# Polochon-street/bliss-rs

Measured on AMD Instinct MI355X. Metric: songs/sec (3-min 22 050 Hz f32) at 1/2/4/8 GPU; HBM GB/s vs roofline, higher is better.
Workload: dtype f32; 1 GPU; configs[1]: batch of 1024 synthetic 3969000-sample (3-min) white-noise f32 PCM buffers per GPU, full 23-feature descriptor set (FeaturesVersion 2); songs_per_gpu=1024, songs_total=1024, features=23, parallelism=single GPU

## Files before the change

bliss-rs_amd/csrc/blissgpu.hip:

```cpp
#include <math.h>
#include <stdio.h>
#include <stdlib.h>
#include <string.h>

#include <algorithm>
#include <atomic>
#include <chrono>
#include <deque>
#include <mutex>
#include <string>
#include <vector>

#include "ctx.hpp"
#include "forest.hpp"

using namespace bg;

namespace {
thread_local std::string g_last_error;

const char* const kKernelNames[K_COUNT] = {
    "fft512_kernel",     "onset_kernel",      "beat_kernel",   "stft8192_kernel", "tune_select_kernel",
    "tune_pass2_kernel", "tune_final_kernel", "chroma_kernel",     "summary_kernel", "assemble_kernel", "pairwise_kernel", "set_distance_kernel", "song_to_song_kernel", "synth_kernel", "rolloff_fix_kernel",
    "dedup_next_kernel", "dedup_walk_kernel", "knn_scan_kernel", "knn_merge_kernel",
// ... 1368 lines not shown
    return BLISSGPU_OK;
}

int blissgpu_debug_fetch(blissgpu_ctx* c, int what, uint32_t song, void* dst, uint64_t max_elems, uint64_t* n_elems) {
    if (!c || !dst) return fail(BLISSGPU_ERR_INVALID, "blissgpu_debug_fetch", "NULL argument");
    CTX_ENTER(c, "blissgpu_debug_fetch");
    if (what == BLISSGPU_DEBUG_FILTER_BANK) {
        if (song > (uint32_t)N_TUNING) return fail(BLISSGPU_ERR_INVALID, "blissgpu_debug_fetch", "tuning slot must be 0..100");
        const uint64_t n = (uint64_t)BANK_ROWS * BANK_PITCH;
        if (n_elems) *n_elems = n;
        const uint64_t k = std::min(n, max_elems);
        HIP_TRY(hipStreamSynchronize(c->stream));
        if (k) HIP_TRY(hipMemcpy(dst, c->chroma_bank + (size_t)song * n, k * sizeof(double), hipMemcpyDeviceToHost));
        return BLISSGPU_OK;
    }
    size_t pos = c->last_songs.size();
    for (size_t i = 0; i < c->last_songs.size(); i++)
        if (c->last_songs[i].row == song) { pos = i; break; }
    if (pos == c->last_songs.size()) return fail(BLISSGPU_ERR_INVALID, "blissgpu_debug_fetch", "no such song in the last chunk");
    HIP_TRY(hipStreamSynchronize(c->stream));
    const SongDesc& d = c->last_songs[pos];
    const Workspace& w = c->last_ws;
    const void* src = nullptr;
    uint64_t n = 0, esz = 4;
    const uint64_t runs = d.ok ? (d.n_b >= (uint32_t)BT_STEP ? (d.n_b - BT_STEP) / BT_STEP + 1 : 0) : 0;
    switch (what) {
        case BLISSGPU_DEBUG_CENTROID: src = w.centroid + d.t_off; n = d.n_t; break;
        case BLISSGPU_DEBUG_ROLLOFF: src = w.rolloff + d.t_off; n = d.n_t; break;
        case BLISSGPU_DEBUG_FLATNESS: src = w.flatness + d.t_off; n = d.n_t; break;
        case BLISSGPU_DEBUG_FLUX: src = w.flux + d.b_off; n = d.n_b; break;
        case BLISSGPU_DEBUG_THRESHOLDED: src = w.thresholded + d.b_off; n = d.n_b; break;
        case BLISSGPU_DEBUG_RUN_BPM: src = w.run_bpm + pos * w.runs_pitch; n = runs; break;
        case BLISSGPU_DEBUG_RUN_COUNT: src = w.run_cnt + pos * w.runs_pitch; n = runs; break;
        case BLISSGPU_DEBUG_SPECTROGRAM: src = w.spec + d.c_off * (size_t)CBINS_PAD; n = (uint64_t)d.n_c * CBINS_PAD; break;
        case BLISSGPU_DEBUG_ENERGY256: src = w.e256 + d.e_off; n = d.n_e; break;
        case BLISSGPU_DEBUG_CROSSINGS256: src = w.zc256 + d.e_off; n = d.n_e; break;
        case BLISSGPU_DEBUG_PITCH_HIST: src = w.hist100 + pos * N_TUNING; n = N_TUNING; break;
        case BLISSGPU_DEBUG_CHROMA:
        case BLISSGPU_DEBUG_INTERVAL:
            if (!w.dbg_chroma || !w.dbg_interval)
                return fail(BLISSGPU_ERR_INVALID, "blissgpu_debug_fetch", "set BLISSGPU_OPT_DEBUG_CHROMA before the analysis");
            esz = 8;
            if (what == BLISSGPU_DEBUG_CHROMA) { src = w.dbg_chroma + d.c_off * 12; n = (uint64_t)d.n_c * 12; }
            else { src = w.dbg_interval + pos * 10; n = 10; }
            break;
        default: return fail(BLISSGPU_ERR_INVALID, "blissgpu_debug_fetch", "unknown tap");
    }
    if (!d.ok) n = 0;
    if (n_elems) *n_elems = n;
    const uint64_t k = std::min(n, max_elems);
    if (k) HIP_TRY(hipMemcpy(dst, src, k * esz, hipMemcpyDeviceToHost));
    return BLISSGPU_OK;
}

}
```

bliss-rs_amd/csrc/internal.hpp:

```cpp
#pragma once
#include <hip/hip_runtime.h>
#include <stdint.h>

#include <vector>

namespace bg {

constexpr uint32_t SAMPLE_RATE = 22050;
constexpr int W512 = 512;
constexpr int HOP_T = 128;
constexpr int HOP_B = 256;
constexpr int W8192 = 8192;
constexpr int HOP_C = 2205;
constexpr int CBINS = W8192 / 2 + 1;
constexpr int CBINS_PAD = 4128;
constexpr int BANK_PITCH = CBINS_PAD;
constexpr int BANK_ROWS = 12;
constexpr int LOUD_W = 1024;
constexpr int MIN_SAMPLES = 8192;
constexpr int N_TUNING = 100;
constexpr int PIP_LO = 57, PIP_HI = 1483;
constexpr int PIP_MAX_PER_FRAME = 714;
constexpr int CAND_BUDGET_PER_FRAME = 48;
#ifndef COARSE_SHIFT
#define COARSE_SHIFT 17
#endif
constexpr uint32_t COARSE_LOW_MASK = (1u << COARSE_SHIFT) - 1u;
constexpr int H1_BINS = 1 << (31 - COARSE_SHIFT);
constexpr int BT_WINLEN = 512, BT_STEP = 128, BT_LAGLEN = 128;
constexpr int BT_PRE_STRIDE = 264;
constexpr int F512_TILE = 512;
constexpr int CH_TILE = 64;
constexpr int STFT_TILE = 16;

struct SongDesc {
    uint64_t pcm_off;
    uint64_t n;
    uint64_t t_off;
    uint64_t b_off;
    uint64_t c_off;
    uint64_t e_off;
    uint32_t n_t;
    uint32_t n_b;
    uint32_t n_f;
    uint32_t n_c;
    uint32_t n_e;
    uint32_t n_l;
    uint32_t row;
    uint32_t ok;
};

struct RollFix {
    float* mags;
    uint32_t cap;
};
constexpr float ROLLOFF_UNPROVEN = -1.0f;

struct TuningState {
    uint32_t n_peaks;
    uint32_t b_lo, b_hi;
    uint32_t below;
    uint32_t n_cand;
    int32_t tuning_idx;
    uint32_t cand_off;
    uint32_t cand_cap;
};

struct TempoState {
    float tempo;
    uint32_t n_bpms;
};

struct DeviceTables {
    const float2* tw8192;
    const float2* tw512;
    const float* hann8192;
    const float* hannz512;
    const double* chroma_bank;
    const float* bt_rwv;
    const float* bt_dfwv;
};

// ... 57 lines not shown
    size_t roll_fix_bytes;
};

struct Batch {
    const float* pcm;
    const SongDesc* songs;
    uint32_t n_songs;
    const uint32_t* pfx_f;
    const uint32_t* pfx_c;
    const uint32_t* pfx_ct;
    const uint32_t* pfx_cw;
    uint32_t tiles_f, tiles_c, tiles_ct, tiles_cw;
    uint64_t total_b;
    uint32_t max_nb;
    uint32_t max_nt;
};

void launch_fft512(const Batch&, const Workspace&, const DeviceTables&, hipStream_t, bool rolloff_exact_all = false, bool seq_flux = false);
void launch_rolloff_fix(const Batch&, const Workspace&, uint64_t total_t, hipStream_t);
void launch_onset(const Batch&, const Workspace&, hipStream_t);
void launch_beat(const Batch&, const Workspace&, const DeviceTables&, hipStream_t);
void launch_beat_acf(const Batch&, const Workspace&, const DeviceTables&, hipStream_t);
void launch_beat_track(const Batch&, const Workspace&, const DeviceTables&, hipStream_t);
void launch_stft8192(const Batch&, const Workspace&, const DeviceTables&, hipStream_t, int shape = 0);
struct SongRange { uint32_t s0, s1, ct0, ct1, cw0, cw1; };
void launch_tune_select(const Batch&, const Workspace&, hipStream_t, const SongRange* r = nullptr);
void launch_tune_pass2(const Batch&, const Workspace&, hipStream_t, const SongRange* r = nullptr);
void launch_tune_final(const Batch&, const Workspace&, hipStream_t, const SongRange* r = nullptr);
void launch_chroma(const Batch&, const Workspace&, const DeviceTables&, hipStream_t, const SongRange* r = nullptr);
void launch_summary(const Batch&, const Workspace&, hipStream_t);
void launch_finalize(const Batch&, const Workspace&, uint32_t features_version, float* d_out, int32_t* d_status,
                     int32_t* dbg_tuning, uint32_t* dbg_nbpms, hipStream_t);
void launch_chroma_bank(double* bank, hipStream_t);
void launch_pcm_convert(const void* in, int sample_format, uint32_t channels, float* out, uint64_t frames, hipStream_t st);
struct SwrPlan;
hipError_t launch_resample(const void* in, int sample_format, uint32_t channels, uint64_t frames, const SwrPlan& plan,
                           const float* d_bank, float* out, uint64_t n_out, hipStream_t st);
void launch_pair_distance(const float* a, const float* b, uint32_t d, int metric, const float* d_M, float* out, hipStream_t st);
void launch_set_distance(const float* seeds, uint32_t n_seeds, const float* cand, uint64_t n, uint32_t d, int metric,
                         const float* M, float* dist, uint32_t* keys, uint32_t* idx, uint32_t* nan_flag, hipStream_t st);
hipError_t sort_pairs_u32(void* tmp, size_t* tmp_bytes, uint32_t* keys_in, uint32_t* keys_out, uint32_t* vals_in,
                          uint32_t* vals_out, uint32_t n, hipStream_t st, uint32_t* sync = nullptr, uint32_t max_coresident = 0);
void launch_song_to_song(const float* seeds, uint32_t n_seeds, const float* cand, uint32_t n, uint32_t d, int metric,
                         const float* M, uint32_t* order, unsigned long long* slots, uint32_t* sync, uint32_t grid,
                         hipStream_t st);
void launch_dedup_next(const float* x, uint64_t n, uint32_t d, const uint32_t* seq, uint32_t len, const uint32_t* meta,
                       int metric, const float* M, float thr, uint32_t* next, uint32_t* bad, hipStream_t st);
void launch_dedup_walk(const float* x, uint64_t n, uint32_t d, const uint32_t* seq, uint32_t len, const uint32_t* meta,
                       int metric, const float* M, float thr, const uint32_t* next, uint32_t* kept, uint64_t* n_kept,
                       uint32_t* nan_flag, uint32_t* bad, hipStream_t st);
struct KnnPlan {
    uint32_t cap;
    uint32_t qb;
    uint32_t n_split;
    uint32_t blocks_per_split;
    uint32_t grid_qb;
    uint64_t part_keys;
};
KnnPlan knn_plan(uint64_t q, uint64_t n, uint32_t k, int n_cus);
void launch_knn_scan(const float* Q, uint64_t q, const float* X, uint32_t n, uint32_t d, int metric, const float* M,
                     int m_is_diag, const uint32_t* skip, uint32_t k, const KnnPlan& p, unsigned long long* part,
                     uint32_t* nan_flag, uint32_t* bad_flag, hipStream_t st);
void launch_knn_merge(const unsigned long long* part, uint64_t q, uint32_t k, const KnnPlan& p, uint32_t* idx, float* dist,
                      hipStream_t st);
constexpr int GROUP_KNN_SEED_TILE = 32;
struct GroupKnnItem {
// ... 37 lines not shown
```

bliss-rs_amd/csrc/kernels_chroma.hip:

```cpp
#include <float.h>
#include <stdlib.h>

#include <type_traits>

#include "device_utils.hpp"
#include "fft_r16.hpp"
#include "internal.hpp"

namespace bg {

typedef double double4_t __attribute__((ext_vector_type(4)));

__device__ __forceinline__ double tuning_of_slot(int slot) {
    return slot >= N_TUNING ? 0.0 : (-50.0 + (100.0 * 0.01 * (double)slot)) / 100.0;
}

__global__ __launch_bounds__(256) void chroma_bank_kernel(double* __restrict__ bank) {
#pragma clang fp contract(off)
    const int slot = blockIdx.y;
    const int k = blockIdx.x * 256 + threadIdx.x;
    if (k >= BANK_PITCH) return;
    double* out = bank + (size_t)slot * BANK_ROWS * BANK_PITCH;
    if (k >= CBINS) {
        for (int r = 0; r < BANK_ROWS; r++) out[(size_t)r * BANK_PITCH + k] = 0.0;
// ... 381 lines not shown
            split_pair_sq(v[R16(j)], (j == 0 && t == 0) ? v[R16(0)] : zm, w, sq_k, sq_m);
            m_lo[j] = mag_from_sq(sq_k);
            m_hi[j] = mag_from_sq(sq_m);
            mx = fmaxf(mx, fmaxf(m_lo[j], m_hi[j]));
        }
        if (t == 0) {
            m_mid = mag_from_sq(split_one_sq(v[R16(8)], v[R16(8)], mk(0.0f, -1.0f)));
            mx = fmaxf(mx, m_mid);
        }
        const bool has_next = fi + 1 < STFT_FRAMES_PER_WG && f + STFT_GROUP < sd.n_c;
        if (has_next) load_frame(f + STFT_GROUP, v);
        mx = wave_max_dpp(mx);
        if constexpr (NARROW) __syncthreads();
        float* mags = reinterpret_cast<float*>(lds);
        float* mags_top = mags + MAGS_TOP_W - 4096;
#pragma unroll
        for (int j = 0; j < 8; j++) {
            mags[t + 256 * j] = m_lo[j];
            if (j == 0 && t == 0) mags_top[4096] = m_hi[0];
            else mags[4096 - (t + 256 * j)] = m_hi[j];
        }
        if (t == 0) mags[2048] = m_mid;
        if (t >= 1 && t < CBINS_PAD - 4096) mags_top[4096 + t] = 0.0f;
        {
            int slot = t >> 6;
            asm volatile("" : "+v"(slot));
            if (lane_id() == 0) red[slot] = mx;
        }
        if (t == 0) peak_count = 0;
        TRACE(10);
        __syncthreads();
        TRACE(11);
        auto store_row = [&]() {
            const __amdgpu_buffer_rsrc_t r_row = __builtin_amdgcn_make_buffer_rsrc(
                (void*)(spec + (sd.c_off + f) * (size_t)CBINS_PAD), 0, CBINS_PAD * 4, 0x00020000);
            const u32x4_t* mags4 = reinterpret_cast<const u32x4_t*>(lds);
#pragma unroll
            for (int i = 0; i < 5; i++) {
                const int q = t + 256 * i;
                if (i < 4 || q < CBINS_PAD / 4) {
                    const u32x4_t val = i < 4 ? mags4[q] : mags4[q - 1024 + MAGS_TOP_W / 4];
                    __builtin_amdgcn_raw_buffer_store_b128(val, r_row, 16u * (uint32_t)q, 0, 2);
                }
            }
        };
        store_row();
        mx = fmaxf(fmaxf(red[0], red[1]), fmaxf(red[2], red[3]));
        if (t == 0) frame_max[sd.c_off + f] = mx;
        if (!have_base) {
            if (t == 0) {
                const uint32_t top = coarse_bin((double)mx);
                lhist_base = top > (uint32_t)(LHIST_BINS * 3 / 4) ? top - (uint32_t)(LHIST_BINS * 3 / 4) : 0u;
            }
            have_base = true;
            __syncthreads();
        }
        TRACE(12);
        const uint32_t lbase = lhist_base;
        __builtin_amdgcn_s_setprio(2);
        const double ref = 0.1 * (double)mx;
        const float thr = ref_floor_f32(ref);
        {
            uint32_t hits = 0;
#pragma unroll
            for (int h = 0; h < 2; h++) {
                float sb3[3], se3[3], sa3[3];
#pragma unroll
                for (int q = 0; q < 3; q++) {
                    const int c = t + 256 * (3 * h + q);
                    sb3[q] = mags[c > 0 ? c - 1 : 0];
                    se3[q] = mags[c];
                    sa3[q] = mags[c + 1];
                }
#pragma unroll
                for (int q = 0; q < 3; q++) {
                    const int j = 3 * h + q, c = t + 256 * j;
                    const uint32_t in_range = (256 * j >= PIP_LO && 256 * j + 255 <= PIP_HI) ? 1u : (uint32_t)(c >= PIP_LO) & (uint32_t)(c <= PIP_HI);
                    const uint32_t pk = in_range & (uint32_t)(sa3[q] <= se3[q]) & (uint32_t)(sb3[q] < se3[q]) & (uint32_t)(se3[q] > thr);
                    hits |= pk << j;
                }
            }
            const uint32_t mine = (uint32_t)__popc(hits);
            const uint32_t incl = wave_scan_incl_u32_dpp(mine);
            uint32_t wbase = 0;
            if (lane_id() == 63) wbase = atomicAdd(&peak_count, incl);
            uint32_t pos = (uint32_t)__builtin_amdgcn_readlane((int)wbase, 63) + incl - mine;
#pragma unroll
            for (int j = 0; j < 6; j++)
                if ((hits >> j) & 1u) peak_list[pos++] = (uint16_t)(t + 256 * j);
            TRACE(13);
            __syncthreads();
            TRACE(14);
            const uint32_t n_peaks = peak_count;
            uint32_t* __restrict__ recs = peak_rec + (sd.c_off + f) * (size_t)PIP_MAX_PER_FRAME;
            if (t == 0) peak_cnt[sd.c_off + f] = n_peaks;
            int c_next = t < n_peaks ? (int)peak_list[t] : PIP_LO;
            for (uint32_t i = t; i < n_peaks; i += 256) {
                const int c = c_next;
                const float sb = mags[c - 1], se = mags[c], sa = mags[c + 1];
                c_next = i + 256 < n_peaks ? (int)peak_list[i + 256] : PIP_LO;
                int pb;
                const uint32_t b = peak_classify(sb, se, sa, ref, c, &pb), rel = b - lbase;
                recs[i] = peak_record(b, pb, c);
                if (rel < (uint32_t)LHIST_BINS) atomicAdd(&lhist[rel], 1u);
                else atomicAdd(&hist[b], 1u);
            }
        }
        __builtin_amdgcn_s_setprio(0);
        if (has_next) {
            load_window();
#pragma unroll
            for (int n1 = 0; n1 < 16; n1++) v[n1] = v[n1] * win[n1];
        }
        TRACE(15);
        __syncthreads();
        TRACE(16);
    }
    TRACE_FLUSH();
    if (have_base) {
        const uint32_t lbase = lhist_base;
        for (int i = t; i < LHIST_BINS; i += 256) {
            const uint32_t c = lhist[i];
            if (c) atomicAdd(&hist[lbase + i], c);
        }
    }
}

// ... 88 lines not shown

__global__ __launch_bounds__(256) void tune_pass2_kernel(const SongDesc* __restrict__ songs, uint32_t n_songs,
                                                         const uint32_t* __restrict__ pfx_ct,
                                                         const float* __restrict__ spec,
                                                         const float* __restrict__ frame_max,
                                                         const uint32_t* __restrict__ peak_rec,
                                                         const uint32_t* __restrict__ peak_cnt,
                                                         TuningState* __restrict__ tuning,
                                                         uint32_t* __restrict__ hist100,
                                                         double* __restrict__ cand_mag,
                                                         uint8_t* __restrict__ cand_pb, uint32_t first_tile) {
    __shared__ uint32_t hist[N_TUNING];
    __shared__ uint32_t slow_list[4][P2_SLOW_CAP];
    const uint32_t bx = blockIdx.x + first_tile;
    const uint32_t s = find_segment(pfx_ct, n_songs, bx);
    const SongDesc sd = songs[s];
    const uint32_t tile = bx - pfx_ct[s];
    const int tid = threadIdx.x, lane = lane_id(), wave = wave_id();
    TuningState* ts = tuning + s;
    const uint32_t b_lo = ts->b_lo, b_hi = ts->b_hi;
    if (ts->n_peaks == 0) return;
    const uint32_t cand_off = ts->cand_off;
    const uint32_t cand_cap = ts->cand_cap;
    const bool pooled = cand_cap != 0;
    if (tid < N_TUNING) hist[tid] = 0;
    __syncthreads();
    uint32_t n_slow = 0;

    auto flush = [&]() {
        for (uint32_t i = lane; i < n_slow; i += WAVE) {
            const uint32_t e = slow_list[wave][i];
            const int c = (int)(e & 0xFFFFu);
            const uint32_t f = tile * CH_TILE + wave + 4 * (e >> 16);
            const float* row = spec + (sd.c_off + f) * (size_t)CBINS_PAD;
            const double ref = 0.1 * (double)frame_max[sd.c_off + f];
            double mag, pitch;
            if (pip_peak_core(row[c - 1], row[c], row[c + 1], ref, c, &mag, &pitch)) {
                const uint32_t b = coarse_bin(mag);
                if (b > b_hi) {
                    atomicAdd(&hist[pitch_bin(pitch)], 1u);
                } else if (b >= b_lo) {
                    const uint32_t slot = atomicAdd(&ts->n_cand, 1u);
                    if (pooled && slot < cand_cap) {
                        cand_mag[cand_off + slot] = mag;
                        cand_pb[cand_off + slot] = (uint8_t)pitch_bin(pitch);
                    }
                }
            }
        }
        __builtin_amdgcn_wave_barrier();
        n_slow = 0;
    };
    uint32_t n_rec_next = 0;
    {
        const uint32_t f0 = tile * CH_TILE + wave;
        if (f0 < sd.n_c) n_rec_next = peak_cnt[sd.c_off + f0];
    }
    for (int i = 0; i < P2_FRAMES_PER_WAVE; i++) {
        const uint32_t f = tile * CH_TILE + wave + 4 * i;
        if (f >= sd.n_c) break;
        const uint32_t n_rec = n_rec_next < (uint32_t)PIP_MAX_PER_FRAME ? n_rec_next : (uint32_t)PIP_MAX_PER_FRAME;
        if (i + 1 < P2_FRAMES_PER_WAVE && f + 4 < sd.n_c) n_rec_next = peak_cnt[sd.c_off + f + 4];
        const uint32_t* __restrict__ recs = peak_rec + (sd.c_off + f) * (size_t)PIP_MAX_PER_FRAME;
        if (n_slow + PIP_MAX_PER_FRAME > P2_SLOW_CAP) flush();
        for (uint32_t j0 = 0; j0 < n_rec; j0 += 4 * WAVE) {
            uint32_t r4[4];
#pragma unroll
            for (int u = 0; u < 4; u++) {
                const uint32_t j = j0 + WAVE * u + lane;
                r4[u] = j < n_rec ? recs[j] : 0xFFFFFFFFu;
            }
#pragma unroll
            for (int u = 0; u < 4; u++) {
                if (j0 + WAVE * u >= n_rec) break;
                const uint32_t j = j0 + WAVE * u + lane;
                bool slow = false;
                uint32_t c = 0;
                if (j < n_rec) {
                    const uint32_t r = r4[u];
                    const uint32_t b = r >> 18, pbf = (r >> 11) & 0x7Fu;
                    c = r & 0x7FFu;
                    if (b > b_hi) {
                        if (pbf) atomicAdd(&hist[pbf - 1], 1u);
                        else slow = true;
                    } else if (b >= b_lo) {
                        slow = true;
                    }
                }
                const uint64_t mask = __ballot(slow);
                if (mask) {
                    if (slow) slow_list[wave][n_slow + (uint32_t)__popcll(mask & ((1ull << lane) - 1ull))] = ((uint32_t)i << 16) | c;
                    n_slow += (uint32_t)__popcll(mask);
                }
            }
        }
    }
// ... 69 lines not shown
    __shared__ unsigned long long s_min_gt;
    const uint32_t s = blockIdx.x + first_song;
    const int tid = threadIdx.x;
    TuningState* ts = tuning + s;
    const SongDesc sd = songs[s];
    if (!sd.ok || ts->n_peaks == 0) return;
    const uint32_t total = ts->n_peaks, nc = ts->n_cand;
    const uint32_t r_lo = (total - 1) / 2, r_hi = total - 1 - r_lo;
    const uint32_t k_lo = r_lo - ts->below, k_hi = r_hi - ts->below;
    const uint32_t b_lo = ts->b_lo, b_hi = ts->b_hi;
    const bool pooled = ts->cand_cap != 0 && nc == ts->cand_cap;
    const double* v = cand_mag + ts->cand_off;
    const uint8_t* pb = cand_pb + ts->cand_off;

    auto for_each = [&](auto&& fn) {
        if (pooled) {
            for (uint32_t i0 = tid; i0 < nc; i0 += 8 * 256) {
                double m8[8];
                int b8[8];
#pragma unroll
                for (int u = 0; u < 8; u++) {
                    const uint32_t i = i0 + 256u * u;
                    m8[u] = i < nc ? v[i] : 0.0;
                    b8[u] = i < nc ? (int)pb[i] : 0;
                }
#pragma unroll
                for (int u = 0; u < 8; u++)
                    if (i0 + 256u * u < nc) fn(m8[u], b8[u]);
            }
        } else {
            for (uint32_t f = 0; f < sd.n_c; f++) {
                const uint32_t n_rec_raw = peak_cnt[sd.c_off + f];
                const uint32_t n_rec = n_rec_raw < (uint32_t)PIP_MAX_PER_FRAME ? n_rec_raw : (uint32_t)PIP_MAX_PER_FRAME;
                const uint32_t* __restrict__ recs = peak_rec + (sd.c_off + f) * (size_t)PIP_MAX_PER_FRAME;
                const float* __restrict__ row = spec + (sd.c_off + f) * (size_t)CBINS_PAD;
                const double ref = 0.1 * (double)frame_max[sd.c_off + f];
                for (uint32_t j = tid; j < n_rec; j += 256) {
                    const uint32_t r = recs[j], b = r >> 18;
                    if (b < b_lo || b > b_hi) continue;
                    const int c = (int)(r & 0x7FFu);
                    double mag, pitch;
                    if (pip_peak_core(row[c - 1], row[c], row[c + 1], ref, c, &mag, &pitch)) fn(mag, pitch_bin(pitch));
                }
            }
        }
    };

    const uint64_t key_lo = block_radix_select(for_each, k_lo, hist, &s_digit, &s_rank, s_wave);
    uint64_t key_hi = key_lo;
    if (k_hi != k_lo) {
        if (tid == 0) { s_cnt_le = 0; s_min_gt = ~0ull; }
        __syncthreads();
        uint32_t cnt = 0;
        unsigned long long mn = ~0ull;
        for_each([&](double mag, int) {
            const uint64_t k = f64_key(mag);
            if (k <= key_lo) cnt++;
            else if (k < mn) mn = k;
        });
        atomicAdd(&s_cnt_le, cnt);
        atomicMin(&s_min_gt, mn);
        __syncthreads();
        if (s_cnt_le <= k_hi) key_hi = s_min_gt;
    }
    double thr;
    {
#pragma clang fp contract(off)
        const double lo = key_f64(key_lo), hi = key_f64(key_hi);
        thr = lo + (hi - lo) / 2.0;
    }
    __syncthreads();
    if (tid < N_TUNING) hist[tid] = hist100[(size_t)s * N_TUNING + tid];
    __syncthreads();
    for_each([&](double mag, int bin) {
        if (mag >= thr) atomicAdd(&hist[bin], 1u);
// ... 11 lines not shown
    const uint32_t s0 = r ? r->s0 : 0, s1 = r ? r->s1 : b.n_songs;
    if (s1 <= s0) return;
    hipLaunchKernelGGL(tune_final_kernel, dim3(s1 - s0), dim3(256), 0, st, b.songs, w.tuning, w.hist100,
                       w.cand_mag, w.cand_pb, w.spec, w.frame_max, w.peak_rec, w.peak_cnt, s0);
}

static constexpr int TMPL_LEN[10] = {2, 2, 2, 2, 2, 2, 3, 3, 3, 3};
static constexpr int TMPL_PC[10][3] = {{0, 1, 0}, {0, 2, 0}, {0, 3, 0}, {0, 4, 0}, {0, 5, 0},
                                       {0, 6, 0}, {0, 4, 7}, {0, 3, 7}, {0, 3, 6}, {0, 4, 8}};

template <int T>
__device__ __forceinline__ double interval_feature(const double (&c)[12]) {
    double acc = 0.0;
#pragma unroll
    for (int shift = 0; shift < 12; shift++) {
        const int r0 = (TMPL_PC[T][0] + shift) % 12, r1 = (TMPL_PC[T][1] + shift) % 12;
        if (TMPL_LEN[T] == 2) {
            acc += c[r0 < r1 ? r0 : r1] * c[r0 < r1 ? r1 : r0];
        } else {
            const int r2 = (TMPL_PC[T][2] + shift) % 12;
            const int lo = r0 < r1 ? (r0 < r2 ? r0 : r2) : (r1 < r2 ? r1 : r2);
            const int hi = r0 > r1 ? (r0 > r2 ? r0 : r2) : (r1 > r2 ? r1 : r2);
            const int mid = r0 + r1 + r2 - lo - hi;
            acc += (c[lo] * c[mid]) * c[hi];
        }
    }
    return acc;
}

__global__ __launch_bounds__(256) void chroma_kernel(const SongDesc* __restrict__ songs, uint32_t n_songs, const uint32_t* __restrict__ pfx_cw,
                              const uint32_t* __restrict__ pfx_ct, const float* __restrict__ spec,
                              const double* __restrict__ bank, const TuningState* __restrict__ tuning,
                              double* __restrict__ chroma_part, double* __restrict__ dbg_chroma, uint32_t first_wg);

void launch_chroma(const Batch& b, const Workspace& w, const DeviceTables& t, hipStream_t st, const SongRange* r) {
    const uint32_t g0 = r ? r->cw0 : 0, g1 = r ? r->cw1 : b.tiles_cw;
    if (g1 <= g0) return;
    hipLaunchKernelGGL(chroma_kernel, dim3(g1 - g0), dim3(256), 0, st, b.songs, b.n_songs, b.pfx_cw, b.pfx_ct, w.spec,
                       t.chroma_bank, w.tuning, w.chroma_part, w.dbg_chroma, g0);
}

#ifndef BG_PROBE_REPLACES_CHROMA_KERNEL
__global__ __launch_bounds__(256) void chroma_kernel(const SongDesc* __restrict__ songs, uint32_t n_songs,
                                                     const uint32_t* __restrict__ pfx_cw,
                                                     const uint32_t* __restrict__ pfx_ct,
                                                     const float* __restrict__ spec,
                                                     const double* __restrict__ bank,
                                                     const TuningState* __restrict__ tuning,
                                                     double* __restrict__ chroma_part,
                                                     double* __restrict__ dbg_chroma, uint32_t first_wg) {
    __shared__ double tile_c[4][4][16][13];
    const uint32_t bx = blockIdx.x + first_wg;
    const uint32_t s = find_segment(pfx_cw, n_songs, bx);
    const SongDesc sd = songs[s];
    const int lane = lane_id(), wave = wave_id();
    const uint32_t tile64 = (bx - pfx_cw[s]) * 4 + wave;
    const uint32_t n_tiles = pfx_ct[s + 1] - pfx_ct[s];
    if (tile64 >= n_tiles) return;
    const int i16 = lane & 15, g = lane >> 4;
    const int tidx = tuning[s].tuning_idx;
    const int slot = (tidx < 0) ? N_TUNING : tidx;
    const uint32_t f0 = tile64 * CH_TILE;

    const double* __restrict__ arow = bank + ((size_t)slot * BANK_ROWS + (i16 < BANK_ROWS ? i16 : BANK_ROWS - 1)) * BANK_PITCH + 8 * g;
    const float* brow[4];
#pragma unroll
    for (int q = 0; q < 4; q++) {
        uint32_t fj = f0 + 16 * q + i16;
        if (fj >= sd.n_c) fj = sd.n_c - 1;
        brow[q] = spec + (sd.c_off + fj) * (size_t)CBINS_PAD + 8 * g;
    }
    double4_t acc[4][2];
#pragma unroll
    for (int q = 0; q < 4; q++) { acc[q][0] = double4_t{0.0, 0.0, 0.0, 0.0}; acc[q][1] = double4_t{0.0, 0.0, 0.0, 0.0}; }
    struct KBlock {
        double4_t a[2];
        float4 b[2][4];
    };
    auto k_load = [&](int k0, KBlock& kb) {
#pragma unroll
        for (int u = 0; u < 2; u++) kb.a[u] = *reinterpret_cast<const double4_t*>(arow + k0 + 4 * u);
#pragma unroll
        for (int q = 0; q < 4; q++)
#pragma unroll
            for (int u = 0; u < 2; u++) kb.b[u][q] = *reinterpret_cast<const float4*>(brow[q] + k0 + 4 * u);
        __builtin_amdgcn_sched_barrier(0);
    };
    auto k_mma = [&](const KBlock& kb) {
#pragma unroll
        for (int u = 0; u < 2; u++) {
#pragma unroll
            for (int q = 0; q < 4; q++) {
                const float4 v = kb.b[u][q];
                const double b0 = (double)v.x * (double)v.x, b1 = (double)v.y * (double)v.y;
                const double b2 = (double)v.z * (double)v.z, b3 = (double)v.w * (double)v.w;
                acc[q][0] = __builtin_amdgcn_mfma_f64_16x16x4f64(kb.a[u].x, b0, acc[q][0], 0, 0, 0);
                acc[q][1] = __builtin_amdgcn_mfma_f64_16x16x4f64(kb.a[u].y, b1, acc[q][1], 0, 0, 0);
                acc[q][0] = __builtin_amdgcn_mfma_f64_16x16x4f64(kb.a[u].z, b2, acc[q][0], 0, 0, 0);
                acc[q][1] = __builtin_amdgcn_mfma_f64_16x16x4f64(kb.a[u].w, b3, acc[q][1], 0, 0, 0);
            }
        }
    };
    constexpr int KBLOCKS = CBINS_PAD / 32;
    static_assert(CBINS_PAD % 32 == 0 && BANK_PITCH == CBINS_PAD && KBLOCKS % 2 == 1, "pairs of blocks and one last block");
    KBlock k0buf, k1buf;
    k_load(0, k0buf);
#pragma unroll 1
    for (int kb = 0; kb + 2 < KBLOCKS; kb += 2) {
        k_load(32 * (kb + 1), k1buf);
        k_mma(k0buf);
        k_load(32 * (kb + 2), k0buf);
        k_mma(k1buf);
    }
    k_mma(k0buf);
#pragma unroll
    for (int q = 0; q < 4; q++) {
        const double4_t cacc = acc[q][0] + acc[q][1];
#pragma unroll
        for (int r = 0; r < 3; r++) tile_c[wave][q][i16][g + 4 * r] = cacc[r];
    }
    __builtin_amdgcn_wave_barrier();
    double feat[10];
#pragma unroll
    for (int t = 0; t < 10; t++) feat[t] = 0.0;
    if (f0 + lane < sd.n_c) {
        double c[12], sum = 0.0;
#pragma unroll
        for (int k = 0; k < 12; k++) { c[k] = tile_c[wave][lane >> 4][lane & 15][k]; sum += fabs(c[k]); }
        if (sum < DBL_MIN) sum = 1.0;
        if (dbg_chroma) {
#pragma unroll
            for (int k = 0; k < 12; k++) dbg_chroma[(sd.c_off + f0 + lane) * 12 + k] = c[k] / sum;
        }
        double esum = 0.0;
#pragma unroll
        for (int k = 0; k < 12; k++) { c[k] = exp((c[k] / sum) * 15.0); esum += fabs(c[k]); }
        if (esum < 0.0001) esum = 1.0;
#pragma unroll
        for (int k = 0; k < 12; k++) c[k] /= esum;
        feat[0] = interval_feature<0>(c); feat[1] = interval_feature<1>(c);
        feat[2] = interval_feature<2>(c); feat[3] = interval_feature<3>(c);
        feat[4] = interval_feature<4>(c); feat[5] = interval_feature<5>(c);
        feat[6] = interval_feature<6>(c); feat[7] = interval_feature<7>(c);
        feat[8] = interval_feature<8>(c); feat[9] = interval_feature<9>(c);
    }
#pragma unroll
    for (int t = 0; t < 10; t++) {
// ... 14 lines not shown
```

bliss-rs_amd/csrc/scheduler.hip:

```cpp
#include <string.h>

#include <algorithm>
#include <chrono>
#include <condition_variable>
#include <numeric>

#include "coalescing_front.hpp"
#include "ctx.hpp"

using namespace bg;

namespace {

inline size_t align_up(size_t x, size_t a) { return (x + a - 1) / a * a; }

void fill_counts(SongDesc& d) {
    const uint64_t n = d.n;
    d.n_t = (uint32_t)((n - W512) / HOP_T + 1);
    d.n_b = (uint32_t)((n - W512) / HOP_B + 1);
    d.n_f = std::max(d.n_t, 2u * d.n_b);
    d.n_c = (uint32_t)ceilf((float)n / (float)HOP_C);
    d.n_e = (uint32_t)((n + 255) / 256);
    d.n_l = (uint32_t)((n + LOUD_W - 1) / LOUD_W);
}

size_t song_ws_bytes(const SongDesc& d) {
    if (!d.ok) return 256;
    size_t b = 0;
    b += (size_t)d.n_t * 12 + (size_t)d.n_b * 8 + (size_t)d.n_e * 8;
    b += (size_t)d.n_c * (CBINS_PAD * 4 + 4);
    b += (size_t)H1_BINS * 4 + N_TUNING * 4 + sizeof(TuningState) + sizeof(TempoState);
    b += (size_t)d.n_c * CAND_BUDGET_PER_FRAME * 9;
    b += (size_t)d.n_c * (PIP_MAX_PER_FRAME * 4 + 4);
    b += ((size_t)d.n_c / CH_TILE + 1) * 80;
    b += ((size_t)d.n_b / BT_STEP + 2) * (8 + BT_PRE_STRIDE * 4);
    return b + 4096;
}

struct Carver {
    uint8_t* base;
    size_t off = 0;
    template <typename T>
    T* take(size_t n) {
        off = align_up(off, 256);
        T* p = reinterpret_cast<T*>(base + off);
        off += n * sizeof(T);
        return p;
    }
};

struct ChunkTotals {
    uint64_t tot_t = 0, tot_b = 0, tot_c = 0, tot_e = 0;
    uint32_t max_nb = 0, max_nt = 0, max_runs = 1;
    uint32_t tiles_ct = 0;
    uint64_t cand_cap = 0;
};

Workspace carve(uint8_t* base, uint32_t ns, const ChunkTotals& t, size_t* bytes) {
    Carver m{base};
    Workspace w{};
    w.centroid = m.take<float>(t.tot_t); w.rolloff = m.take<float>(t.tot_t); w.flatness = m.take<float>(t.tot_t);
    w.flux = m.take<float>(t.tot_b); w.thresholded = m.take<float>(t.tot_b);
    w.e256 = m.take<float>(t.tot_e); w.zc256 = m.take<uint32_t>(t.tot_e);
    static_assert((size_t)(CBINS_PAD + PIP_MAX_PER_FRAME) * 4 * HOP_T >= (size_t)256 * 4 * HOP_C,
                  "the borrowed stretch must hold one 256-word entry per timbral frame: bytes per chroma frame x samples per "
                  "timbral frame >= bytes per entry x samples per chroma frame");
    w.spec = m.take<float>(t.tot_c * CBINS_PAD + 64);
    w.peak_rec = m.take<uint32_t>(t.tot_c * PIP_MAX_PER_FRAME);
    w.roll_fix_bytes = (size_t)(reinterpret_cast<uint8_t*>(w.peak_rec + t.tot_c * PIP_MAX_PER_FRAME) - reinterpret_cast<uint8_t*>(w.spec));
    w.frame_max = m.take<float>(t.tot_c);
    w.roll_fix = m.take<RollFix>(1);
    w.h1 = m.take<uint32_t>((size_t)ns * H1_BINS); w.hist100 = m.take<uint32_t>((size_t)ns * N_TUNING);
    w.tuning = m.take<TuningState>(ns);
    w.peak_cnt = m.take<uint32_t>(t.tot_c);
    w.cand_mag = m.take<double>(t.cand_cap); w.cand_pb = m.take<uint8_t>(t.cand_cap);
    w.cand_cursor = m.take<uint32_t>(4);
    w.cand_cap = (uint32_t)t.cand_cap;
    w.chroma_part = m.take<double>((size_t)t.tiles_ct * 10 + 16);
    w.tempo = m.take<TempoState>(ns);
    w.run_bpm = m.take<float>((size_t)ns * t.max_runs); w.run_cnt = m.take<uint32_t>((size_t)ns * t.max_runs);
    w.runs_pitch = t.max_runs;
    w.bt_pre = m.take<float>((size_t)(t.tot_b / BT_STEP + ns + 1) * BT_PRE_STRIDE);
    w.summary = m.take<float>((size_t)ns * 16);
    *bytes = m.off + 4096;
    return w;
}

int ensure_mask_stream(blissgpu_ctx* c, int cus) {
    cus = std::max(1, std::min(cus, c->n_cus));
    if (c->mask_stream && c->mask_cus == cus) return BLISSGPU_OK;
    if (c->mask_stream) { (void)hipStreamSynchronize(c->mask_stream); (void)hipStreamDestroy(c->mask_stream); c->mask_stream = nullptr; }
    std::vector<uint32_t> mask((size_t)(c->n_cus + 31) / 32, 0u);
    for (int i = 0; i < cus; i++) mask[(size_t)i / 32] |= 1u << (i % 32);
    HIP_TRY(hipExtStreamCreateWithCUMask(&c->mask_stream, (uint32_t)mask.size(), mask.data()));
    c->mask_cus = cus;
    return BLISSGPU_OK;
}

int ensure_slot_events(ChunkSlot& s) {
    if (s.ev_free) return BLISSGPU_OK;
    hipEvent_t* evs[] = {&s.ev_start, &s.ev_fork, &s.ev_stft, &s.ev_sel, &s.ev_tune, &s.ev_sum, &s.ev_chroma, &s.ev_desc, &s.ev_free, &s.ev_acf, &s.ev_beat};
    for (hipEvent_t* e : evs) HIP_TRY(hipEventCreateWithFlags(e, hipEventDisableTiming));
    for (hipEvent_t& e : s.ev_piece) HIP_TRY(hipEventCreateWithFlags(&e, hipEventDisableTiming));
    return BLISSGPU_OK;
}

int chunk_front(blissgpu_ctx* c, ChunkSlot& slot, const float* d_pcm, SongDesc* songs, uint32_t ns, bool only_chunk) {
    int rc = ensure_slot_events(slot);
    if (rc) return rc;
    std::vector<uint32_t> pfx_f(ns + 1, 0), pfx_c(ns + 1, 0), pfx_ct(ns + 1, 0), pfx_cw(ns + 1, 0);
    ChunkTotals t;
    for (uint32_t i = 0; i < ns; i++) {
        SongDesc& d = songs[i];
        d.t_off = t.tot_t; d.b_off = t.tot_b; d.c_off = t.tot_c; d.e_off = t.tot_e;
        if (d.ok) {
            t.tot_t += d.n_t; t.tot_b += d.n_b; t.tot_c += d.n_c; t.tot_e += d.n_e;
            t.max_nb = std::max(t.max_nb, d.n_b);
            t.max_nt = std::max(t.max_nt, d.n_t);
            t.max_runs = std::max(t.max_runs, d.n_b / BT_STEP + 1);
        }
        pfx_f[i + 1] = pfx_f[i] + (d.ok ? (d.n_f + F512_TILE - 1) / F512_TILE : 0);
        pfx_c[i + 1] = pfx_c[i] + (d.ok ? 4 * ((d.n_c + 4 * STFT_TILE - 1) / (4 * STFT_TILE)) : 0);
        pfx_ct[i + 1] = pfx_ct[i] + (d.ok ? (d.n_c + CH_TILE - 1) / CH_TILE : 0);
        pfx_cw[i + 1] = pfx_cw[i] + (d.ok ? (d.n_c + 4 * CH_TILE - 1) / (4 * CH_TILE) : 0);
    }
    t.tiles_ct = pfx_ct[ns];
    t.cand_cap = std::min<uint64_t>(t.tot_c * (uint64_t)c->cand_budget, 0xFFFFFF00ull) + 64;

    const size_t desc_bytes = align_up(ns * sizeof(SongDesc), 256) + 4 * align_up((ns + 1) * 4, 256) + 256;
    size_t need = 0;
    (void)carve(nullptr, ns, t, &need);
    if ((rc = slot.desc.ensure(desc_bytes))) return rc;
    if ((rc = slot.slab.ensure(need))) return rc;
    if (slot.used) HIP_TRY(hipEventSynchronize(slot.ev_desc));
    if ((rc = slot.h_desc.ensure(desc_bytes))) return rc;

    hipStream_t st = c->stream, sb = c->serial ? c->stream : c->aux_stream, sc = c->serial ? c->stream : c->chr_stream;
    const bool multi = !c->serial;
    if (slot.used && multi) HIP_TRY(hipStreamWaitEvent(st, slot.ev_free, 0));

    uint8_t* h = slot.h_desc.p;
    size_t o = 0;
    const size_t o_songs = o; memcpy(h + o, songs, ns * sizeof(SongDesc)); o = align_up(o + ns * sizeof(SongDesc), 256);
    const size_t o_f = o; memcpy(h + o, pfx_f.data(), (ns + 1) * 4); o = align_up(o + (ns + 1) * 4, 256);
    const size_t o_c = o; memcpy(h + o, pfx_c.data(), (ns + 1) * 4); o = align_up(o + (ns + 1) * 4, 256);
    const size_t o_ct = o; memcpy(h + o, pfx_ct.data(), (ns + 1) * 4); o = align_up(o + (ns + 1) * 4, 256);
    const size_t o_cw = o; memcpy(h + o, pfx_cw.data(), (ns + 1) * 4); o = align_up(o + (ns + 1) * 4, 256);
// ... 846 lines not shown
```

Measured before the change: 27820 songs/sec.

## Store chroma spectrogram in K-blocked 64-frame tiles and pad peak records

Replaces the row-major spectrogram (one CBINS_PAD row per frame) with per-song 64-frame tiles laid out as 32-bin K-blocks, so the chroma contraction reads contiguous float4 runs across its 16-frame subgroups. The contraction now skips missing 16-frame subtiles of a partial tile via compile-time specialisations instead of clamping to the last frame. Peak records get a padded pitch of 736 words. All spectrogram readers (pass-2, tuning fallback, debug tap via a new un-tiling kernel) are updated to the new indexing. Partial tiles now occupy a full tile of memory, which slightly raises the workspace footprint.

```diff
diff --git a/bliss-rs_amd/csrc/blissgpu.hip b/bliss-rs_amd/csrc/blissgpu.hip
--- a/bliss-rs_amd/csrc/blissgpu.hip
+++ b/bliss-rs_amd/csrc/blissgpu.hip
@@ -1424,7 +1424,7 @@
         case BLISSGPU_DEBUG_THRESHOLDED: src = w.thresholded + d.b_off; n = d.n_b; break;
         case BLISSGPU_DEBUG_RUN_BPM: src = w.run_bpm + pos * w.runs_pitch; n = runs; break;
         case BLISSGPU_DEBUG_RUN_COUNT: src = w.run_cnt + pos * w.runs_pitch; n = runs; break;
-        case BLISSGPU_DEBUG_SPECTROGRAM: src = w.spec + d.c_off * (size_t)CBINS_PAD; n = (uint64_t)d.n_c * CBINS_PAD; break;
+        case BLISSGPU_DEBUG_SPECTROGRAM: n = (uint64_t)d.n_c * CBINS_PAD; break;
         case BLISSGPU_DEBUG_ENERGY256: src = w.e256 + d.e_off; n = d.n_e; break;
         case BLISSGPU_DEBUG_CROSSINGS256: src = w.zc256 + d.e_off; n = d.n_e; break;
         case BLISSGPU_DEBUG_PITCH_HIST: src = w.hist100 + pos * N_TUNING; n = N_TUNING; break;
@@ -1441,6 +1441,19 @@
     if (!d.ok) n = 0;
     if (n_elems) *n_elems = n;
     const uint64_t k = std::min(n, max_elems);
+    if (k && what == BLISSGPU_DEBUG_SPECTROGRAM) {
+        float* rows = nullptr;
+        hipError_t e = hipMalloc((void**)&rows, k * sizeof(float));
+        if (e != hipSuccess) { (void)hipGetLastError(); return fail(BLISSGPU_ERR_OOM, "hipMalloc(spectrogram tap)", hipGetErrorString(e)); }
+        launch_spec_rows(w.spec + (size_t)d.c_tile * SPEC_TILE_FLOATS, rows, k, c->stream);
+        e = hipGetLastError();
+        if (e == hipSuccess) e = hipMemcpyAsync(dst, rows, k * sizeof(float), hipMemcpyDeviceToHost, c->stream);
+        const hipError_t es = hipStreamSynchronize(c->stream);
+        (void)hipFree(rows);
+        if (e == hipSuccess) e = es;
+        if (e != hipSuccess) return fail(BLISSGPU_ERR_HIP, "blissgpu_debug_fetch", hipGetErrorString(e));
+        return BLISSGPU_OK;
+    }
     if (k) HIP_TRY(hipMemcpy(dst, src, k * esz, hipMemcpyDeviceToHost));
     return BLISSGPU_OK;
 }
diff --git a/bliss-rs_amd/csrc/internal.hpp b/bliss-rs_amd/csrc/internal.hpp
--- a/bliss-rs_amd/csrc/internal.hpp
+++ b/bliss-rs_amd/csrc/internal.hpp
@@ -21,6 +21,7 @@
 constexpr int N_TUNING = 100;
 constexpr int PIP_LO = 57, PIP_HI = 1483;
 constexpr int PIP_MAX_PER_FRAME = 714;
+constexpr int PEAK_REC_PITCH = 736;
 constexpr int CAND_BUDGET_PER_FRAME = 48;
 #ifndef COARSE_SHIFT
 #define COARSE_SHIFT 17
@@ -32,6 +33,12 @@
 constexpr int F512_TILE = 512;
 constexpr int CH_TILE = 64;
 constexpr int STFT_TILE = 16;
+constexpr int SPEC_KBLOCKS = CBINS_PAD / 32;
+constexpr int SPEC_KBLOCK_FLOATS = CH_TILE * 32;
+constexpr int SPEC_TILE_FLOATS = SPEC_KBLOCKS * SPEC_KBLOCK_FLOATS;
+__host__ __device__ __forceinline__ constexpr uint32_t spec_word(uint32_t r, uint32_t c) {
+    return (c >> 5) * (uint32_t)SPEC_KBLOCK_FLOATS + r * 32u + (c & 31u);
+}
 
 struct SongDesc {
     uint64_t pcm_off;
@@ -48,6 +55,8 @@
     uint32_t n_l;
     uint32_t row;
     uint32_t ok;
+    uint32_t c_tile;
+    uint32_t pad_;
 };
 
 struct RollFix {
@@ -171,6 +180,7 @@
 void launch_finalize(const Batch&, const Workspace&, uint32_t features_version, float* d_out, int32_t* d_status,
                      int32_t* dbg_tuning, uint32_t* dbg_nbpms, hipStream_t);
 void launch_chroma_bank(double* bank, hipStream_t);
+void launch_spec_rows(const float* tiles, float* rows, uint64_t n_elems, hipStream_t);
 void launch_pcm_convert(const void* in, int sample_format, uint32_t channels, float* out, uint64_t frames, hipStream_t st);
 struct SwrPlan;
 hipError_t launch_resample(const void* in, int sample_format, uint32_t channels, uint64_t frames, const SwrPlan& plan,
diff --git a/bliss-rs_amd/csrc/kernels_chroma.hip b/bliss-rs_amd/csrc/kernels_chroma.hip
--- a/bliss-rs_amd/csrc/kernels_chroma.hip
+++ b/bliss-rs_amd/csrc/kernels_chroma.hip
@@ -437,15 +437,17 @@
         __syncthreads();
         TRACE(11);
         auto store_row = [&]() {
-            const __amdgpu_buffer_rsrc_t r_row = __builtin_amdgcn_make_buffer_rsrc(
-                (void*)(spec + (sd.c_off + f) * (size_t)CBINS_PAD), 0, CBINS_PAD * 4, 0x00020000);
+            const __amdgpu_buffer_rsrc_t r_tile = __builtin_amdgcn_make_buffer_rsrc(
+                (void*)(spec + (sd.c_tile + (f / CH_TILE)) * (size_t)SPEC_TILE_FLOATS), 0, SPEC_TILE_FLOATS * 4, 0x00020000);
             const u32x4_t* mags4 = reinterpret_cast<const u32x4_t*>(lds);
+            const uint32_t voff = ((uint32_t)t >> 3) * (uint32_t)(SPEC_KBLOCK_FLOATS * 4) + ((uint32_t)t & 7u) * 16u;
+            const uint32_t soff = (f % CH_TILE) * 128u;
 #pragma unroll
             for (int i = 0; i < 5; i++) {
                 const int q = t + 256 * i;
                 if (i < 4 || q < CBINS_PAD / 4) {
                     const u32x4_t val = i < 4 ? mags4[q] : mags4[q - 1024 + MAGS_TOP_W / 4];
-                    __builtin_amdgcn_raw_buffer_store_b128(val, r_row, 16u * (uint32_t)q, 0, 2);
+                    __builtin_amdgcn_raw_buffer_store_b128(val, r_tile, voff, soff + (uint32_t)i * (32u * SPEC_KBLOCK_FLOATS * 4u), 2);
                 }
             }
         };
@@ -497,7 +499,7 @@
             __syncthreads();
             TRACE(14);
             const uint32_t n_peaks = peak_count;
-            uint32_t* __restrict__ recs = peak_rec + (sd.c_off + f) * (size_t)PIP_MAX_PER_FRAME;
+            uint32_t* __restrict__ recs = peak_rec + (sd.c_off + f) * (size_t)PEAK_REC_PITCH;
             if (t == 0) peak_cnt[sd.c_off + f] = n_peaks;
             int c_next = t < n_peaks ? (int)peak_list[t] : PIP_LO;
             for (uint32_t i = t; i < n_peaks; i += 256) {
@@ -652,10 +654,11 @@
             const uint32_t e = slow_list[wave][i];
             const int c = (int)(e & 0xFFFFu);
             const uint32_t f = tile * CH_TILE + wave + 4 * (e >> 16);
-            const float* row = spec + (sd.c_off + f) * (size_t)CBINS_PAD;
+            const float* tl = spec + (sd.c_tile + tile) * (size_t)SPEC_TILE_FLOATS;
+            const uint32_t r = f % CH_TILE;
             const double ref = 0.1 * (double)frame_max[sd.c_off + f];
             double mag, pitch;
-            if (pip_peak_core(row[c - 1], row[c], row[c + 1], ref, c, &mag, &pitch)) {
+            if (pip_peak_core(tl[spec_word(r, c - 1)], tl[spec_word(r, c)], tl[spec_word(r, c + 1)], ref, c, &mag, &pitch)) {
                 const uint32_t b = coarse_bin(mag);
                 if (b > b_hi) {
                     atomicAdd(&hist[pitch_bin(pitch)], 1u);
@@ -681,7 +684,7 @@
         if (f >= sd.n_c) break;
         const uint32_t n_rec = n_rec_next < (uint32_t)PIP_MAX_PER_FRAME ? n_rec_next : (uint32_t)PIP_MAX_PER_FRAME;
         if (i + 1 < P2_FRAMES_PER_WAVE && f + 4 < sd.n_c) n_rec_next = peak_cnt[sd.c_off + f + 4];
-        const uint32_t* __restrict__ recs = peak_rec + (sd.c_off + f) * (size_t)PIP_MAX_PER_FRAME;
+        const uint32_t* __restrict__ recs = peak_rec + (sd.c_off + f) * (size_t)PEAK_REC_PITCH;
         if (n_slow + PIP_MAX_PER_FRAME > P2_SLOW_CAP) flush();
         for (uint32_t j0 = 0; j0 < n_rec; j0 += 4 * WAVE) {
             uint32_t r4[4];
@@ -817,15 +820,16 @@
             for (uint32_t f = 0; f < sd.n_c; f++) {
                 const uint32_t n_rec_raw = peak_cnt[sd.c_off + f];
                 const uint32_t n_rec = n_rec_raw < (uint32_t)PIP_MAX_PER_FRAME ? n_rec_raw : (uint32_t)PIP_MAX_PER_FRAME;
-                const uint32_t* __restrict__ recs = peak_rec + (sd.c_off + f) * (size_t)PIP_MAX_PER_FRAME;
-                const float* __restrict__ row = spec + (sd.c_off + f) * (size_t)CBINS_PAD;
+                const uint32_t* __restrict__ recs = peak_rec + (sd.c_off + f) * (size_t)PEAK_REC_PITCH;
+                const float* __restrict__ tl = spec + (sd.c_tile + f / CH_TILE) * (size_t)SPEC_TILE_FLOATS;
+                const uint32_t rs = f % CH_TILE;
                 const double ref = 0.1 * (double)frame_max[sd.c_off + f];
                 for (uint32_t j = tid; j < n_rec; j += 256) {
                     const uint32_t r = recs[j], b = r >> 18;
                     if (b < b_lo || b > b_hi) continue;
                     const int c = (int)(r & 0x7FFu);
                     double mag, pitch;
-                    if (pip_peak_core(row[c - 1], row[c], row[c + 1], ref, c, &mag, &pitch)) fn(mag, pitch_bin(pitch));
+                    if (pip_peak_core(tl[spec_word(rs, c - 1)], tl[spec_word(rs, c)], tl[spec_word(rs, c + 1)], ref, c, &mag, &pitch)) fn(mag, pitch_bin(pitch));
                 }
             }
         }
@@ -903,6 +907,18 @@
                               const uint32_t* __restrict__ pfx_ct, const float* __restrict__ spec,
                               const double* __restrict__ bank, const TuningState* __restrict__ tuning,
                               double* __restrict__ chroma_part, double* __restrict__ dbg_chroma, uint32_t first_wg);
+
+__global__ __launch_bounds__(256) void spec_rows_kernel(const float* __restrict__ tiles, float* __restrict__ rows, uint64_t n_elems) {
+    const uint64_t i = (uint64_t)blockIdx.x * 256 + threadIdx.x;
+    if (i >= n_elems) return;
+    const uint32_t f = (uint32_t)(i / CBINS_PAD), c = (uint32_t)(i % CBINS_PAD);
+    rows[i] = tiles[(size_t)(f / CH_TILE) * SPEC_TILE_FLOATS + spec_word(f % CH_TILE, c)];
+}
+
+void launch_spec_rows(const float* tiles, float* rows, uint64_t n_elems, hipStream_t st) {
+    if (n_elems == 0) return;
+    hipLaunchKernelGGL(spec_rows_kernel, dim3((uint32_t)((n_elems + 255) / 256)), dim3(256), 0, st, tiles, rows, n_elems);
+}
 
 void launch_chroma(const Batch& b, const Workspace& w, const DeviceTables& t, hipStream_t st, const SongRange* r) {
     const uint32_t g0 = r ? r->cw0 : 0, g1 = r ? r->cw1 : b.tiles_cw;
@@ -934,13 +950,8 @@
     const uint32_t f0 = tile64 * CH_TILE;
 
     const double* __restrict__ arow = bank + ((size_t)slot * BANK_ROWS + (i16 < BANK_ROWS ? i16 : BANK_ROWS - 1)) * BANK_PITCH + 8 * g;
-    const float* brow[4];
-#pragma unroll
-    for (int q = 0; q < 4; q++) {
-        uint32_t fj = f0 + 16 * q + i16;
-        if (fj >= sd.n_c) fj = sd.n_c - 1;
-        brow[q] = spec + (sd.c_off + fj) * (size_t)CBINS_PAD + 8 * g;
-    }
+    const float* __restrict__ brow = spec + (sd.c_tile + tile64) * (size_t)SPEC_TILE_FLOATS + i16 * 32 + 8 * g;
+    const uint32_t n_sub = min(4u, (sd.n_c - f0 + 15u) / 16u);
     double4_t acc[4][2];
 #pragma unroll
     for (int q = 0; q < 4; q++) { acc[q][0] = double4_t{0.0, 0.0, 0.0, 0.0}; acc[q][1] = double4_t{0.0, 0.0, 0.0, 0.0}; }
@@ -948,20 +959,21 @@
         double4_t a[2];
         float4 b[2][4];
     };
-    auto k_load = [&](int k0, KBlock& kb) {
-#pragma unroll
-        for (int u = 0; u < 2; u++) kb.a[u] = *reinterpret_cast<const double4_t*>(arow + k0 + 4 * u);
-#pragma unroll
-        for (int q = 0; q < 4; q++)
-#pragma unroll
-            for (int u = 0; u < 2; u++) kb.b[u][q] = *reinterpret_cast<const float4*>(brow[q] + k0 + 4 * u);
+    auto k_load = [&](auto nq, int kblk, KBlock& kb) {
+#pragma unroll
+        for (int u = 0; u < 2; u++) kb.a[u] = *reinterpret_cast<const double4_t*>(arow + 32 * kblk + 4 * u);
+#pragma unroll
+        for (int q = 0; q < decltype(nq)::value; q++)
+#pragma unroll
+            for (int u = 0; u < 2; u++)
+                kb.b[u][q] = *reinterpret_cast<const float4*>(brow + (size_t)kblk * SPEC_KBLOCK_FLOATS + q * (16 * 32) + 4 * u);
         __builtin_amdgcn_sched_barrier(0);
     };
-    auto k_mma = [&](const KBlock& kb) {
+    auto k_mma = [&](auto nq, const KBlock& kb) {
 #pragma unroll
         for (int u = 0; u < 2; u++) {
 #pragma unroll
-            for (int q = 0; q < 4; q++) {
+            for (int q = 0; q < decltype(nq)::value; q++) {
                 const float4 v = kb.b[u][q];
                 const double b0 = (double)v.x * (double)v.x, b1 = (double)v.y * (double)v.y;
                 const double b2 = (double)v.z * (double)v.z, b3 = (double)v.w * (double)v.w;
@@ -974,16 +986,23 @@
     };
     constexpr int KBLOCKS = CBINS_PAD / 32;
     static_assert(CBINS_PAD % 32 == 0 && BANK_PITCH == CBINS_PAD && KBLOCKS % 2 == 1, "pairs of blocks and one last block");
-    KBlock k0buf, k1buf;
-    k_load(0, k0buf);
+    static_assert(KBLOCKS == SPEC_KBLOCKS, "the stored tile has one K-block per block of this loop");
+    auto contract = [&](auto nq) {
+        KBlock k0buf, k1buf;
+        k_load(nq, 0, k0buf);
 #pragma unroll 1
-    for (int kb = 0; kb + 2 < KBLOCKS; kb += 2) {
-        k_load(32 * (kb + 1), k1buf);
-        k_mma(k0buf);
-        k_load(32 * (kb + 2), k0buf);
-        k_mma(k1buf);
-    }
-    k_mma(k0buf);
+        for (int kb = 0; kb + 2 < KBLOCKS; kb += 2) {
+            k_load(nq, kb + 1, k1buf);
+            k_mma(nq, k0buf);
+            k_load(nq, kb + 2, k0buf);
+            k_mma(nq, k1buf);
+        }
+        k_mma(nq, k0buf);
+    };
+    if (n_sub == 4) contract(std::integral_constant<int, 4>{});
+    else if (n_sub == 3) contract(std::integral_constant<int, 3>{});
+    else if (n_sub == 2) contract(std::integral_constant<int, 2>{});
+    else contract(std::integral_constant<int, 1>{});
 #pragma unroll
     for (int q = 0; q < 4; q++) {
         const double4_t cacc = acc[q][0] + acc[q][1];
diff --git a/bliss-rs_amd/csrc/scheduler.hip b/bliss-rs_amd/csrc/scheduler.hip
--- a/bliss-rs_amd/csrc/scheduler.hip
+++ b/bliss-rs_amd/csrc/scheduler.hip
@@ -28,10 +28,10 @@
     if (!d.ok) return 256;
     size_t b = 0;
     b += (size_t)d.n_t * 12 + (size_t)d.n_b * 8 + (size_t)d.n_e * 8;
-    b += (size_t)d.n_c * (CBINS_PAD * 4 + 4);
+    b += ((size_t)d.n_c + CH_TILE - 1) / CH_TILE * ((size_t)SPEC_TILE_FLOATS * 4) + (size_t)d.n_c * 4;
     b += (size_t)H1_BINS * 4 + N_TUNING * 4 + sizeof(TuningState) + sizeof(TempoState);
     b += (size_t)d.n_c * CAND_BUDGET_PER_FRAME * 9;
-    b += (size_t)d.n_c * (PIP_MAX_PER_FRAME * 4 + 4);
+    b += (size_t)d.n_c * (PEAK_REC_PITCH * 4 + 4);
     b += ((size_t)d.n_c / CH_TILE + 1) * 80;
     b += ((size_t)d.n_b / BT_STEP + 2) * (8 + BT_PRE_STRIDE * 4);
     return b + 4096;
@@ -62,12 +62,12 @@
     w.centroid = m.take<float>(t.tot_t); w.rolloff = m.take<float>(t.tot_t); w.flatness = m.take<float>(t.tot_t);
     w.flux = m.take<float>(t.tot_b); w.thresholded = m.take<float>(t.tot_b);
     w.e256 = m.take<float>(t.tot_e); w.zc256 = m.take<uint32_t>(t.tot_e);
-    static_assert((size_t)(CBINS_PAD + PIP_MAX_PER_FRAME) * 4 * HOP_T >= (size_t)256 * 4 * HOP_C,
+    static_assert((size_t)(CBINS_PAD + PEAK_REC_PITCH) * 4 * HOP_T >= (size_t)256 * 4 * HOP_C,
                   "the borrowed stretch must hold one 256-word entry per timbral frame: bytes per chroma frame x samples per "
                   "timbral frame >= bytes per entry x samples per chroma frame");
-    w.spec = m.take<float>(t.tot_c * CBINS_PAD + 64);
-    w.peak_rec = m.take<uint32_t>(t.tot_c * PIP_MAX_PER_FRAME);
-    w.roll_fix_bytes = (size_t)(reinterpret_cast<uint8_t*>(w.peak_rec + t.tot_c * PIP_MAX_PER_FRAME) - reinterpret_cast<uint8_t*>(w.spec));
+    w.spec = m.take<float>((size_t)t.tiles_ct * SPEC_TILE_FLOATS + 64);
+    w.peak_rec = m.take<uint32_t>(t.tot_c * PEAK_REC_PITCH);
+    w.roll_fix_bytes = (size_t)(reinterpret_cast<uint8_t*>(w.peak_rec + t.tot_c * PEAK_REC_PITCH) - reinterpret_cast<uint8_t*>(w.spec));
     w.frame_max = m.take<float>(t.tot_c);
     w.roll_fix = m.take<RollFix>(1);
     w.h1 = m.take<uint32_t>((size_t)ns * H1_BINS); w.hist100 = m.take<uint32_t>((size_t)ns * N_TUNING);
@@ -113,6 +113,7 @@
     for (uint32_t i = 0; i < ns; i++) {
         SongDesc& d = songs[i];
         d.t_off = t.tot_t; d.b_off = t.tot_b; d.c_off = t.tot_c; d.e_off = t.tot_e;
+        d.c_tile = pfx_ct[i];
         if (d.ok) {
             t.tot_t += d.n_t; t.tot_b += d.n_b; t.tot_c += d.n_c; t.tot_e += d.n_e;
             t.max_nb = std::max(t.max_nb, d.n_b);
```

After: 27800 songs/sec. No clear change (-0.1%).
